# anilkeshwani/speech-integration

Measured on AMD Instinct MI355X. Metric: train_tokens_per_sec, higher is better.
Workload: dtype bf16; 1 GPU; Llama-3.2-1B +5000 DSUs (V=133258), SFT step fwd+bwd+AdamW, seq_len=2048, batch=8/GPU, grad_accum=1, 16 layers, random-init weights, MLS-shaped synthetic DSU sequences; global_batch=8, seq_len=2048, parallelism=dp1

## Files before the change

speech-integration_amd/csrc/attn_mfma.h:

```cpp
#pragma once
#include <type_traits>
#include "common_hip.h"

namespace {

__device__ __forceinline__ bf16x4 unrope4(bf16x4 v, f32x4 cs) {
    const float x0 = (float)v[0], x1 = (float)v[1], x2 = (float)v[2], x3 = (float)v[3];
    bf16x4 o;
    o[0] = (bf16_t)(x0 * cs[0] + x1 * cs[1]);
    o[1] = (bf16_t)(x1 * cs[0] - x0 * cs[1]);
    o[2] = (bf16_t)(x2 * cs[2] + x3 * cs[3]);
    o[3] = (bf16_t)(x3 * cs[2] - x2 * cs[3]);
    return o;
}
__device__ __forceinline__ bf16x4 unrope4(bf16x4 v, const float* __restrict__ tb, int d0) {
    return unrope4(v, *reinterpret_cast<const f32x4*>(tb + d0));
}

__device__ __forceinline__ void block_to_work(int n_blocks, int n_pairs, int& rank, int& pair) {
    const int i = (int)blockIdx.x;
    if (n_pairs % 8 == 0) {
        const int ppx = n_pairs / 8, xcd = i & 7, j = i >> 3;
        rank = j / ppx;
        pair = xcd * ppx + j % ppx;
    } else {
        rank = i % n_blocks;
        pair = i / n_blocks;
    }
}

__device__ __forceinline__ void ring_barrier() { asm volatile("s_waitcnt lgkmcnt(0)\n\ts_barrier" ::: "memory"); }

#ifdef ATTN_TRACE
constexpr int TRACE_MAX = 8192;
__device__ unsigned long long g_attn_trace[3][TRACE_MAX][6];
#define TRACE_BEGIN() const unsigned long long tr_t0_ = __builtin_amdgcn_s_memrealtime(); unsigned long long tr_ta_ = 0, tr_tb_ = 0
#define TRACE_LOOP_BEGIN() tr_ta_ = __builtin_amdgcn_s_memrealtime()
#define TRACE_LOOP_END() tr_tb_ = __builtin_amdgcn_s_memrealtime()
#define TRACE_END(k, work)                                                                                                        \
    if (threadIdx.x == 0 && blockIdx.x < TRACE_MAX) {                                                                             \
        unsigned hw_, xcc_;                                                                                                       \
        asm volatile("s_getreg_b32 %0, hwreg(HW_REG_HW_ID)" : "=s"(hw_));                                                        \
        asm volatile("s_getreg_b32 %0, hwreg(HW_REG_XCC_ID)" : "=s"(xcc_));                                                      \
        g_attn_trace[k][blockIdx.x][0] = tr_t0_;                                                                                  \
        g_attn_trace[k][blockIdx.x][1] = __builtin_amdgcn_s_memrealtime();                                                        \
        g_attn_trace[k][blockIdx.x][2] = ((unsigned long long)xcc_ << 32) | hw_;                                                  \
        g_attn_trace[k][blockIdx.x][3] = (unsigned long long)(work);                                                              \
        g_attn_trace[k][blockIdx.x][4] = tr_ta_;                                                                                  \
        g_attn_trace[k][blockIdx.x][5] = tr_tb_;                                                                                  \
    }
#else
#define TRACE_BEGIN()
#define TRACE_LOOP_BEGIN()
#define TRACE_LOOP_END()
#define TRACE_END(k, work)
#endif

constexpr int HD = 64;
constexpr float LOG2E = 1.4426950408889634f;

__device__ __forceinline__ int rowmap(int r, int h) { return (r & 3) + 8 * (r >> 2) + 4 * h; }

enum { SWZ_ROW = 0, SWZ_TR = 1, SWZ_DUAL = 2 };
template <int SWZ> __device__ __forceinline__ int swz(int row) {
    if (SWZ == SWZ_ROW) return (row >> 1) & 7;
    if (SWZ == SWZ_TR) return ((row >> 1) & 1) << 2;
    return (((row >> 1) & 1) << 2) | ((row >> 2) & 3);
}

template <int SWZ> __device__ __forceinline__ bf16x8 frag_row(const char* tile, int row_base, int ks, int lane) {
    const int row = row_base + (lane & 31);
    const int chunk = (2 * ks + (lane >> 5)) ^ swz<SWZ>(row);
    return *reinterpret_cast<const bf16x8*>(tile + row * 128 + chunk * 16);
}

template <int SWZ> __device__ __forceinline__ bf16x8 frag_tr(const char* tile, int kbase, int cbase, int lane) {
    const int G = lane >> 4, h = G >> 1, i = lane & 15, q = i >> 2, p = i & 3;
    const int chunk = ((cbase + 16 * (G & 1)) >> 3) + (p >> 1);
    const int r0 = kbase + 4 * h + q, r1 = r0 + 8;
    const char* a0 = tile + r0 * 128 + ((chunk ^ swz<SWZ>(r0)) * 16) + 8 * (p & 1);
    const char* a1 = tile + r1 * 128 + ((chunk ^ swz<SWZ>(r1)) * 16) + 8 * (p & 1);
    s16x4 lo = __builtin_amdgcn_ds_read_tr16_b64_v4i16((__attribute__((address_space(3))) s16x4*)a0);
    s16x4 hi = __builtin_amdgcn_ds_read_tr16_b64_v4i16((__attribute__((address_space(3))) s16x4*)a1);
    typedef __attribute__((ext_vector_type(8))) short s16x8;
    s16x8 r = __builtin_shufflevector(lo, hi, 0, 1, 2, 3, 4, 5, 6, 7);
    return __builtin_bit_cast(bf16x8, r);
}

template <int SWZ> __device__ __forceinline__ s16x4 frag_tr_half(const char* tile, int kbase, int cbase, int lane, int half) {
    const int G = lane >> 4, h = G >> 1, i = lane & 15, q = i >> 2, p = i & 3;
    const int chunk = ((cbase + 16 * (G & 1)) >> 3) + (p >> 1);
    const int r = kbase + 4 * h + q + 8 * half;
    const char* a = tile + r * 128 + ((chunk ^ swz<SWZ>(r)) * 16) + 8 * (p & 1);
    return __builtin_amdgcn_ds_read_tr16_b64_v4i16((__attribute__((address_space(3))) s16x4*)a);
}

__device__ __forceinline__ bf16x8 acc_frag(const f32x16& a, int s) {
    bf16x8 f;
#pragma unroll
    for (int j = 0; j < 8; ++j) f[j] = (bf16_t)a[8 * s + j];
    return f;
}

__device__ __forceinline__ bf16x8 scale_frag(bf16x8 v, float s) {
#pragma unroll
    for (int j = 0; j < 8; ++j) v[j] = (bf16_t)((float)v[j] * s);
    return v;
}

template <int ROWS, int NTHR> struct TileStage {
    static constexpr int N = ROWS * 8 / NTHR;
    u32x4 r[N];
    __device__ __forceinline__ void load(const bf16_t* g, int64_t ld, int tid) {
#pragma unroll
        for (int i = 0; i < N; ++i) {
            const int c = tid + i * NTHR;
            r[i] = *reinterpret_cast<const u32x4*>(g + (int64_t)(c >> 3) * ld + (c & 7) * 8);
        }
    }
    template <int SWZ> __device__ __forceinline__ void store(char* tile, int tid) const {
#pragma unroll
        for (int i = 0; i < N; ++i) {
            const int c = tid + i * NTHR, row = c >> 3, chunk = (c & 7) ^ swz<SWZ>(row);
            *reinterpret_cast<u32x4*>(tile + row * 128 + chunk * 16) = r[i];
        }
    }
};

typedef __attribute__((address_space(3))) char lds_c;
constexpr unsigned BUF_RSRC_WORD3 = 0x00020000u;
__device__ __forceinline__ u32x4 buffer_rsrc(const void* base) {
    const uint64_t a = (uint64_t)(uintptr_t)base;
    u32x4 r;
    r[0] = __builtin_amdgcn_readfirstlane((unsigned)a);
    r[1] = __builtin_amdgcn_readfirstlane((unsigned)(a >> 32) & 0xffffu);
    r[2] = 0x7fffffffu;
    r[3] = BUF_RSRC_WORD3;
    return r;
}
__device__ __forceinline__ void dma16(unsigned lds_dst, unsigned voff, u32x4 rs, unsigned soff) {
    asm volatile("s_mov_b32 m0, %0\n\ts_nop 0\n\tbuffer_load_dwordx4 %1, %2, %3 offen lds" ::"s"(lds_dst), "v"(voff), "s"(rs), "s"(soff) : "memory");
}
__device__ __forceinline__ void dma4(unsigned lds_dst, unsigned voff, u32x4 rs, unsigned soff) {
    asm volatile("s_mov_b32 m0, %0\n\ts_nop 0\n\tbuffer_load_dword %1, %2, %3 offen lds" ::"s"(lds_dst), "v"(voff), "s"(rs), "s"(soff) : "memory");
}

#ifndef ATTN_NW
#define ATTN_NW 4
#endif
constexpr int ANW = ATTN_NW, ANP = 8 / ATTN_NW;
template <int SWZ_K, int SWZ_V> struct KvTileDma {
    u32x4 rs;
    unsigned vk[ANP], vv[ANP];
    unsigned lds_piece;
    unsigned tile_bytes;
    __device__ __forceinline__ void init(const bf16_t* kbase, int64_t ld, int kv_cols, const char* smem, int wave, int lane) {
        rs = buffer_rsrc(kbase);
#pragma unroll
        for (int p = 0; p < ANP; ++p) {
            const int row = (p * ANW + wave) * 8 + (lane >> 3);
            vk[p] = (unsigned)((row * ld + ((lane & 7) ^ swz<SWZ_K>(row)) * 8) * 2);
            vv[p] = (unsigned)((row * ld + kv_cols + ((lane & 7) ^ swz<SWZ_V>(row)) * 8) * 2);
        }
        lds_piece = __builtin_amdgcn_readfirstlane((unsigned)(uintptr_t)(lds_c*)smem + (unsigned)wave * 1024u);
        tile_bytes = (unsigned)(64 * ld * 2);
    }
    __device__ __forceinline__ void tile(int t, unsigned slot_bytes) const {
        const unsigned soff = (unsigned)t * tile_bytes;
#pragma unroll
        for (int p = 0; p < ANP; ++p) {
            dma16(lds_piece + slot_bytes + p * ANW * 1024, vk[p], rs, soff);
            dma16(lds_piece + slot_bytes + 8192 + p * ANW * 1024, vv[p], rs, soff);
        }
    }
    __device__ __forceinline__ void piece(int t, unsigned slot_bytes, int i) const {
        const unsigned soff = (unsigned)t * tile_bytes;
        const int p = i >> 1;
        if (i & 1) dma16(lds_piece + slot_bytes + 8192 + p * ANW * 1024, vv[p], rs, soff);
        else dma16(lds_piece + slot_bytes + p * ANW * 1024, vk[p], rs, soff);
    }
};

struct RowTileDma {
    u32x4 rs;
    unsigned voff[2];
    unsigned step;
    __device__ __forceinline__ void init(const bf16_t* base, int64_t ld, int lane) {
        rs = buffer_rsrc(base);
#pragma unroll
        for (int par = 0; par < 2; ++par)
            voff[par] = (unsigned)(((lane >> 3) * ld + ((lane & 7) ^ (lane >> 4) ^ (4 * par)) * 8) * 2);
        step = (unsigned)(8 * ld * 2);
    }
    __device__ __forceinline__ void request(int i, unsigned lds_tile) const { dma16(lds_tile + i * 1024, voff[i & 1], rs, (unsigned)i * step); }
};

__device__ __forceinline__ unsigned pack_bf16(float a, float b) {
    typedef __attribute__((ext_vector_type(2))) __bf16 bf16x2_;
    bf16x2_ v;
    v[0] = (bf16_t)a;
    v[1] = (bf16_t)b;
    return __builtin_bit_cast(unsigned, v);
}

}

struct AttnBwdArgs {
    const void* qkv; int64_t ld; const void *out, *dout; const float* lse; void* dqkv; float* delta;
    const int32_t *doc_start, *doc_end; const float* rope; int64_t table_len; const int32_t* positions;
    int64_t batch, seq; int n_heads, n_kv; void* workspace; int64_t workspace_bytes;
    const int32_t *plan_dev, *plan_header;
    hipStream_t stream;
};
```

speech-integration_amd/csrc/common_hip.h:

```cpp
#pragma once
#include <hip/hip_runtime.h>
#include <stdint.h>
#include <stdio.h>
#include "../../include/ssi_hip.h"

typedef __bf16 bf16_t;
typedef __attribute__((ext_vector_type(2))) float f32x2;
typedef __attribute__((ext_vector_type(4))) float f32x4;
typedef __attribute__((ext_vector_type(16))) float f32x16;
typedef __attribute__((ext_vector_type(4))) __bf16 bf16x4;
typedef __attribute__((ext_vector_type(8))) __bf16 bf16x8;
typedef __attribute__((ext_vector_type(4))) short s16x4;
typedef __attribute__((ext_vector_type(4))) unsigned int u32x4;
typedef __attribute__((ext_vector_type(2))) unsigned int u32x2;

#define SSI_WAVE 64

void ssi_set_error(const char* fmt, ...);

#define SSI_CHECK_ARG(cond)                                                                  \
    do {                                                                                     \
        if (!(cond)) {                                                                       \
            ssi_set_error("%s:%d: argument check failed: %s", __FILE__, __LINE__, #cond);    \
            return SSI_ERR_ARG;                                                              \
        }                                                                                    \
    } while (0)

#define SSI_LAUNCH_CHECK()                                                                   \
    do {                                                                                     \
        hipError_t e_ = hipGetLastError();                                                   \
        if (e_ != hipSuccess) {                                                              \
            ssi_set_error("%s:%d: launch failed: %s", __FILE__, __LINE__, hipGetErrorString(e_)); \
            return SSI_ERR_HIP + (int)e_;                                                    \
        }                                                                                    \
    } while (0)

static inline int64_t ssi_cdiv(int64_t a, int64_t b) { return (a + b - 1) / b; }
static inline int64_t ssi_align_up(int64_t a, int64_t b) { return ssi_cdiv(a, b) * b; }

template <typename T> __device__ __forceinline__ float to_f32(T v);
template <> __device__ __forceinline__ float to_f32<float>(float v) { return v; }
template <> __device__ __forceinline__ float to_f32<bf16_t>(bf16_t v) { return (float)v; }
template <typename T> __device__ __forceinline__ T from_f32(float v);
template <> __device__ __forceinline__ float from_f32<float>(float v) { return v; }
template <> __device__ __forceinline__ bf16_t from_f32<bf16_t>(float v) { return (bf16_t)v; }

template <typename T> __device__ __forceinline__ float ssi_sigmoid(float x);
template <> __device__ __forceinline__ float ssi_sigmoid<float>(float x) { return 1.f / (1.f + expf(-x)); }
template <> __device__ __forceinline__ float ssi_sigmoid<bf16_t>(float x) {
    return __builtin_amdgcn_rcpf(1.f + __builtin_amdgcn_exp2f(x * -1.44269504088896f));
}
template <typename T> __device__ __forceinline__ float ssi_silu(float x);
template <> __device__ __forceinline__ float ssi_silu<float>(float x) { return x / (1.f + expf(-x)); }
template <> __device__ __forceinline__ float ssi_silu<bf16_t>(float x) { return x * ssi_sigmoid<bf16_t>(x); }
template <typename T> __device__ __forceinline__ void ssi_swiglu_bwd_elem(float gf, float uf, float df, float& dgate, float& dup) {
#pragma clang fp contract(off)
    const float sig = ssi_sigmoid<T>(gf);
    const float one_minus = 1.f - sig;
    const float t = 1.f + gf * one_minus;
    dup = df * (gf * sig);
    dgate = (df * uf) * (sig * t);
}

__device__ __forceinline__ void ssi_rope_pair(float x0, float x1, float c, float s, float& o0, float& o1) {
#pragma clang fp contract(off)
    o0 = x0 * c - x1 * s;
    o1 = x1 * c + x0 * s;
}

template <typename T> struct Vec16;
template <> struct Vec16<float> {
    static constexpr int N = 4;
    f32x4 v;
    __device__ __forceinline__ float get(int i) const { return v[i]; }
    __device__ __forceinline__ void set(int i, float x) { v[i] = x; }
};
template <> struct Vec16<bf16_t> {
    static constexpr int N = 8;
    bf16x8 v;
    __device__ __forceinline__ float get(int i) const { return (float)v[i]; }
    __device__ __forceinline__ void set(int i, float x) { v[i] = (bf16_t)x; }
};
template <typename T> __device__ __forceinline__ Vec16<T> load16(const T* p) {
    Vec16<T> r;
    r.v = *reinterpret_cast<const decltype(r.v)*>(p);
    return r;
}
template <typename T> __device__ __forceinline__ void store16(T* p, const Vec16<T>& r) {
    *reinterpret_cast<decltype(r.v)*>(p) = r.v;
}

template <typename T> __device__ __forceinline__ Vec16<T> load16_nt(const T* p) {
    Vec16<T> r;
    r.v = __builtin_nontemporal_load(reinterpret_cast<const decltype(r.v)*>(p));
    return r;
}
template <typename T> __device__ __forceinline__ void store16_nt(T* p, const Vec16<T>& r) {
    __builtin_nontemporal_store(r.v, reinterpret_cast<decltype(r.v)*>(p));
}

__device__ __forceinline__ float wave_sum(float v) {
#pragma unroll
    for (int o = 32; o > 0; o >>= 1) v += __shfl_xor(v, o, 64);
    return v;
}
__device__ __forceinline__ float wave_max(float v) {
#pragma unroll
    for (int o = 32; o > 0; o >>= 1) v = fmaxf(v, __shfl_xor(v, o, 64));
    return v;
}
__device__ __forceinline__ float block_sum(float v, float* red) {
    v = wave_sum(v);
    const int w = threadIdx.x >> 6, l = threadIdx.x & 63, nw = (blockDim.x + 63) >> 6;
    __syncthreads();
    if (l == 0) red[w] = v;
    __syncthreads();
    float t = (l < nw) ? red[l] : 0.f;
    t = wave_sum(t);
    return t;
}
__device__ __forceinline__ float block_max(float v, float* red) {
    v = wave_max(v);
    const int w = threadIdx.x >> 6, l = threadIdx.x & 63, nw = (blockDim.x + 63) >> 6;
    __syncthreads();
    if (l == 0) red[w] = v;
    __syncthreads();
    float t = (l < nw) ? red[l] : -INFINITY;
    t = wave_max(t);
    return t;
}

template <bool ENABLED, int N, bool FENCED = false> struct PhaseStamps {
    unsigned long long begin = __builtin_readcyclecounter(), last = begin, total[N] = {};
    __device__ __forceinline__ void reset() {
        if (FENCED) __builtin_amdgcn_sched_barrier(0);
        last = __builtin_readcyclecounter();
        if (FENCED) __builtin_amdgcn_sched_barrier(0);
    }
    __device__ __forceinline__ void tick(int i) {
        const unsigned long long prev = last;
        reset();
        total[i] += last - prev;
    }
};
template <int N, bool FENCED> struct PhaseStamps<false, N, FENCED> {
    __device__ __forceinline__ void reset() {}
    __device__ __forceinline__ void tick(int) {}
};

int ssi_get_impl();

bool ssi_gemm_mfma_supported(int layout, int64_t M, int64_t N, int64_t K, const void* A, int64_t lda, const void* B,
                             int64_t ldb, const void* C, int64_t ldc, const void* R);
int ssi_gemm_mfma_bf16(int layout, int64_t M, int64_t N, int64_t K, const void* A, int64_t lda, const void* B,
                       int64_t ldb, void* C, int64_t ldc, const void* R, float alpha, const float* alpha_dev,
                       int accumulate, void* stream);
int ssi_gemm_mfma_bf16_splitk(int layout, int64_t M, int64_t N, int64_t K, const void* A, int64_t lda, const void* B,
                              int64_t ldb, void* C, int64_t ldc, const void* R, float alpha, const float* alpha_dev,
                              int accumulate, int splits, float* slabs, void* stream);
bool ssi_gemm_mfma_bf16_batched(int layout, int batch, int64_t M, int64_t N, int64_t K, const void* A, int64_t lda, int64_t bsA, const void* B,
                                int64_t ldb, int64_t bsB, void* C, int64_t ldc, int64_t bsC, float alpha, const float* alpha_dev, int accumulate,
                                void* stream, int* rc);
void ssi_gemm_mfma_set_dynamic_tiles(int on);
bool ssi_gemm_rope_mfma(int64_t M, int64_t N, int64_t K, const void* A, int64_t lda, const void* B, int64_t ldb, void* C, int64_t ldc,
                        const float* rope, const int32_t* positions, int64_t seq, int64_t rot_cols, void* stream, int* rc);
bool ssi_gemm_swiglu_supported(int64_t M, int64_t inter, int64_t K, const void* p0, const void* p1, const void* p2, const void* p3,
                               int64_t ld0, int64_t ld1, int64_t ld2, int64_t ld3);
int ssi_gemm_swiglu_fwd_mfma(int64_t M, int64_t inter, int64_t K, const void* X, int64_t ldx, const void* W13, int64_t ldw,
                             void* GU, int64_t ldgu, void* ACT, int64_t ldact, void* stream);
int ssi_gemm_swiglu_bwd_mfma(int layout, int64_t M, int64_t inter, int64_t K, const void* DY, int64_t lddy, const void* W2, int64_t ldw,
                             const void* GU, int64_t ldgu, void* DGU, int64_t lddgu, void* stream);
bool ssi_gemm_swiglu_bwd_nn_supported(int64_t K, int64_t lddy, int64_t ldw);

bool ssi_gemm_f32_mfma_supported(int layout, int64_t M, int64_t N, int64_t K, const void* A, int64_t lda, const void* B,
                                 int64_t ldb, const void* C, int64_t ldc, const void* R);
int ssi_gemm_f32_mfma(int layout, int64_t M, int64_t N, int64_t K, const void* A, int64_t lda, const void* B, int64_t ldb,
                      void* C, int64_t ldc, const void* R, float alpha, const float* alpha_dev, int accumulate,
                      void* stream);

bool ssi_attn_mfma_supported(int64_t ld, int64_t batch, int64_t seq, int n_heads, int n_kv, int head_dim, int dtype);
void ssi_attn_note_dispatch(int v);
int ssi_attn_bwd_mfma(const void* qkv, int64_t ld, const void* out, const void* dout, const float* lse, void* dqkv,
                      float* delta, const int32_t* doc_start, const int32_t* doc_end, const float* rope, int64_t table_len,
                      const int32_t* positions, int64_t batch, int64_t seq, int n_heads, int n_kv, void* workspace, int64_t workspace_bytes,
                      const int32_t* plan_dev, const int32_t* host_plan_header, void* stream);
int ssi_attn_fwd_mfma(const void* qkv, int64_t ld, void* out, float* lse, const int32_t* doc_start, int64_t batch, int64_t seq,
                      int n_heads, int n_kv, void* stream);
int64_t ssi_attn_mfma_bwd_workspace_bytes(int64_t batch, int64_t seq, int n_heads, int n_kv);

#define SSI_DISPATCH_DTYPE(dtype, ...)                           \
    do {                                                         \
        if ((dtype) == SSI_F32) {                                \
            using T = float;                                     \
            __VA_ARGS__;                                         \
        } else if ((dtype) == SSI_BF16) {                        \
            using T = bf16_t;                                    \
            __VA_ARGS__;                                         \
        } else {                                                 \
            ssi_set_error("unsupported dtype %d", (int)(dtype)); \
            return SSI_ERR_ARG;                                  \
        }                                                        \
    } while (0)
```

speech-integration_amd/csrc/embed_ce.hip:

```cpp
#include "common_hip.h"

template <typename T>
__global__ __launch_bounds__(256) void embed_fwd_kernel(const int64_t* __restrict__ tokens, const T* __restrict__ table,
                                                        T* __restrict__ out, int64_t n_tok, int dim, int64_t vocab) {
    constexpr int N = Vec16<T>::N;
    const int nvec = dim / N;
    for (int64_t t = blockIdx.x; t < n_tok; t += gridDim.x) {
        const int64_t tok = tokens[t];
        const bool ok = tok >= 0 && tok < vocab;
        for (int v = threadIdx.x; v < nvec; v += 256) {
            Vec16<T> a;
            if (ok) a = load16(table + tok * dim + v * N);
            else
#pragma unroll
                for (int i = 0; i < N; ++i) a.set(i, 0.f);
            store16(out + t * dim + v * N, a);
        }
    }
}

extern "C" int ssi_embed_fwd(const int64_t* tokens, const void* table, void* out, int64_t n_tok, int64_t dim,
                             int64_t vocab, int dtype, void* stream) {
    if (n_tok == 0) return SSI_OK;
    SSI_CHECK_ARG(tokens && table && out && n_tok > 0 && dim > 0 && dim % 8 == 0 && vocab > 0);
    const unsigned grid = (unsigned)(n_tok < 65536 ? n_tok : 65536);
    SSI_DISPATCH_DTYPE(dtype, hipLaunchKernelGGL(embed_fwd_kernel<T>, dim3(grid), dim3(256), 0, (hipStream_t)stream, tokens,
                                                 (const T*)table, (T*)out, n_tok, (int)dim, vocab));
    SSI_LAUNCH_CHECK();
    return SSI_OK;
}

__global__ __launch_bounds__(256) void embed_index_kernel(const int64_t* __restrict__ tokens, int64_t n_tok, int64_t vocab,
                                                          int* __restrict__ first, int* __restrict__ count) {
    const int64_t t = (int64_t)blockIdx.x * 256 + threadIdx.x;
    if (t >= n_tok) return;
    const int64_t tok = tokens[t];
    if (tok < 0 || tok >= vocab) return;
    atomicMin(&first[tok], (int)t);
    atomicAdd(&count[tok], 1);
}

template <typename T, int MAXV>
__global__ __launch_bounds__(256) void embed_bwd_kernel(const int64_t* __restrict__ tokens, const T* __restrict__ dout,
                                                        T* __restrict__ dtable, int64_t n_tok, int dim, int64_t vocab,
                                                        const int* __restrict__ first, const int* __restrict__ count) {
    constexpr int N = Vec16<T>::N;
    const int lane = threadIdx.x & 63;
    const int64_t t0 = (int64_t)blockIdx.x * 4 + (threadIdx.x >> 6);
    if (t0 >= n_tok) return;
    const int64_t tok = tokens[t0];
    if (tok < 0 || tok >= vocab) return;
    if (first[tok] != (int)t0) return;
    const int need = count[tok];
    const int nvec = dim / N;
    float acc[MAXV][N];
#pragma unroll
    for (int k = 0; k < MAXV; ++k)
#pragma unroll
        for (int i = 0; i < N; ++i) acc[k][i] = 0.f;
    constexpr int SCAN = 8, ROWS = 8;
    __shared__ int hits_lds[4][64 * SCAN];
    int* hits = hits_lds[threadIdx.x >> 6];
    int found = 0;
    for (int64_t base0 = (t0 / 64) * 64; base0 < n_tok && found < need; base0 += 64 * SCAN) {
        int64_t tk[SCAN];
#pragma unroll
        for (int u = 0; u < SCAN; ++u) {
            const int64_t idx = base0 + 64 * u + lane;
            tk[u] = tokens[idx < n_tok ? idx : n_tok - 1];
        }
        int n = 0;
#pragma unroll
        for (int u = 0; u < SCAN; ++u) {
            const int64_t idx = base0 + 64 * u + lane;
            const bool hit = idx < n_tok && idx >= t0 && tk[u] == tok;
            const unsigned long long mask = __ballot(hit);
            if (hit) hits[n + __popcll(mask & ((1ull << lane) - 1ull))] = (int)(idx - base0);
            n += __popcll(mask);
        }
        __builtin_amdgcn_s_waitcnt(0xc07f);
        if (n == 1) {
            const T* src = dout + (base0 + hits[0]) * dim;
#pragma unroll
            for (int k = 0; k < MAXV; ++k) {
                const int v = lane + k * 64;
                const Vec16<T> r = load16(src + (v < nvec ? v : nvec - 1) * N);
#pragma unroll
                for (int i = 0; i < N; ++i) acc[k][i] += v < nvec ? r.get(i) : 0.f;
            }
        } else
        for (int h0 = 0; h0 < n; h0 += ROWS) {
            int pos[ROWS];
#pragma unroll
            for (int u = 0; u < ROWS; ++u) pos[u] = hits[h0 + u < n ? h0 + u : n - 1];
            Vec16<T> a[ROWS][MAXV];
#pragma unroll
            for (int u = 0; u < ROWS; ++u) {
                const T* src = dout + (base0 + pos[u]) * dim;
#pragma unroll
                for (int k = 0; k < MAXV; ++k) {
                    const int v = lane + k * 64;
                    a[u][k] = load16(src + (v < nvec ? v : nvec - 1) * N);
                }
            }
            __builtin_amdgcn_sched_barrier(0);
#pragma unroll
            for (int u = 0; u < ROWS; ++u) {
                const bool row_ok = h0 + u < n;
#pragma unroll
                for (int k = 0; k < MAXV; ++k) {
                    const bool ok = row_ok && lane + k * 64 < nvec;
#pragma unroll
                    for (int i = 0; i < N; ++i) acc[k][i] += ok ? a[u][k].get(i) : 0.f;
                }
            }
        }
        found += n;
    }
    T* dst = dtable + tok * dim;
#pragma unroll
    for (int k = 0; k < MAXV; ++k) {
        const int v = lane + k * 64;
        if (v < nvec) {
            Vec16<T> a = load16(dst + v * N);
#pragma unroll
            for (int i = 0; i < N; ++i) a.set(i, a.get(i) + acc[k][i]);
            store16(dst + v * N, a);
        }
    }
}

static inline int64_t embed_ws_vocab_slots(int64_t vocab) { return ssi_align_up(vocab, 64); }
extern "C" int64_t ssi_embed_bwd_workspace_bytes(int64_t vocab) { return 2 * embed_ws_vocab_slots(vocab) * (int64_t)sizeof(int); }

template <typename T>
static int launch_embed_bwd(const int64_t* tokens, const T* dout, T* dtable, int64_t n_tok, int dim, int64_t vocab,
                            const int* first, const int* count, hipStream_t st) {
    const int64_t vec_per_lane = ssi_cdiv(dim / Vec16<T>::N, 64);
    const dim3 grid((unsigned)ssi_cdiv(n_tok, 4));
    if (vec_per_lane <= 1) hipLaunchKernelGGL((embed_bwd_kernel<T, 1>), grid, dim3(256), 0, st, tokens, dout, dtable, n_tok, dim, vocab, first, count);
    else if (vec_per_lane <= 2) hipLaunchKernelGGL((embed_bwd_kernel<T, 2>), grid, dim3(256), 0, st, tokens, dout, dtable, n_tok, dim, vocab, first, count);
    else if (vec_per_lane <= 4) hipLaunchKernelGGL((embed_bwd_kernel<T, 4>), grid, dim3(256), 0, st, tokens, dout, dtable, n_tok, dim, vocab, first, count);
    else if (vec_per_lane <= 8) hipLaunchKernelGGL((embed_bwd_kernel<T, 8>), grid, dim3(256), 0, st, tokens, dout, dtable, n_tok, dim, vocab, first, count);
    else { ssi_set_error("embed_bwd: dim %d too large", dim); return SSI_ERR_UNSUPPORTED; }
    return SSI_OK;
}

extern "C" int ssi_embed_bwd(const int64_t* tokens, const void* dout, void* dtable, int64_t n_tok, int64_t dim,
                             int64_t vocab, int dtype, void* workspace, int64_t workspace_bytes, void* stream) {
    if (n_tok == 0) return SSI_OK;
    SSI_CHECK_ARG(tokens && dout && dtable && n_tok > 0 && n_tok < (1LL << 31) && dim > 0 && dim % 8 == 0 && vocab > 0);
    if (!workspace || workspace_bytes < ssi_embed_bwd_workspace_bytes(vocab)) { ssi_set_error("embed_bwd: workspace too small"); return SSI_ERR_WORKSPACE; }
    auto st = (hipStream_t)stream;
    int* first = (int*)workspace;
    int* count = first + embed_ws_vocab_slots(vocab);
    hipError_t e = hipMemsetAsync(first, 0x7f, embed_ws_vocab_slots(vocab) * sizeof(int), st);
    if (e == hipSuccess) e = hipMemsetAsync(count, 0, embed_ws_vocab_slots(vocab) * sizeof(int), st);
    if (e != hipSuccess) { ssi_set_error("embed_bwd: memset failed: %s", hipGetErrorString(e)); return SSI_ERR_HIP + (int)e; }
    hipLaunchKernelGGL(embed_index_kernel, dim3((unsigned)ssi_cdiv(n_tok, 256)), dim3(256), 0, st, tokens, n_tok, vocab, first, count);
    SSI_LAUNCH_CHECK();
    int rc = SSI_OK;
    SSI_DISPATCH_DTYPE(dtype, rc = launch_embed_bwd<T>(tokens, (const T*)dout, (T*)dtable, n_tok, (int)dim, vocab, first, count, st));
    if (rc) return rc;
    SSI_LAUNCH_CHECK();
    return SSI_OK;
}

template <typename T>
__global__ __launch_bounds__(512) void ce_fwd_kernel(T* __restrict__ logits, int64_t ld, const int64_t* __restrict__ labels,
                                                     int64_t vocab, int64_t ignore_index, float* __restrict__ row_loss,
                                                     float* __restrict__ row_lse, int write_grad, const float* __restrict__ row_weight) {
    constexpr int N = Vec16<T>::N;
    __shared__ float red[16];
    const int64_t row = blockIdx.x;
    T* lr = logits + row * ld;
    const int64_t label = labels[row];
    const bool valid = label != ignore_index && label >= 0 && label < vocab;
    const int64_t nvec = ld / N;
    if (!valid) {
        if (threadIdx.x == 0) { row_loss[row] = 0.f; if (row_lse) row_lse[row] = 0.f; }
        if (write_grad) {
            Vec16<T> z;
#pragma unroll
            for (int i = 0; i < N; ++i) z.set(i, 0.f);
            for (int64_t v = threadIdx.x; v < nvec; v += 512) store16(lr + v * N, z);
        }
        return;
    }
    float m = -INFINITY, s = 0.f;
    for (int64_t v = threadIdx.x; v < nvec; v += 512) {
        Vec16<T> a = load16(lr + v * N);
        float lm = -INFINITY;
#pragma unroll
        for (int i = 0; i < N; ++i) if (v * N + i < vocab) lm = fmaxf(lm, a.get(i));
        if (lm > m) { s *= expf(m - lm); m = lm; }
#pragma unroll
        for (int i = 0; i < N; ++i) if (v * N + i < vocab) s += expf(a.get(i) - m);
    }
    const float gm = block_max(m, red);
    s = (m == -INFINITY) ? 0.f : s * expf(m - gm);
    const float gs = block_sum(s, red);
    const float lse = gm + logf(gs);
    const float w = row_weight ? row_weight[row] : 1.f;
    if (threadIdx.x == 0) {
        row_loss[row] = w * (lse - to_f32<T>(lr[label]));
        if (row_lse) row_lse[row] = lse;
    }
    if (!write_grad) return;
    __syncthreads();
    for (int64_t v = threadIdx.x; v < nvec; v += 512) {
        Vec16<T> a = load16(lr + v * N), o;
#pragma unroll
        for (int i = 0; i < N; ++i) {
            const int64_t c = v * N + i;
            float g = 0.f;
            if (c < vocab) g = w * (expf(a.get(i) - lse) - (c == label ? 1.f : 0.f));
            o.set(i, g);
        }
        store16(lr + v * N, o);
    }
}

template <int NCH, bool write_grad>
__global__ __launch_bounds__(1024, 4) void ce_row_bf16_kernel(bf16_t* __restrict__ logits, int64_t ld, const int64_t* __restrict__ labels,
                                                              int64_t rows, int64_t vocab, int64_t ignore_index,
                                                              float* __restrict__ row_loss, float* __restrict__ row_lse,
                                                              const float* __restrict__ row_weight) {
    __shared__ float red[16];
    constexpr float LOG2E = 1.44269504088896340736f;
    constexpr int CHUNK = 8192;
    const int tid = threadIdx.x;
    const int voff = tid * 16;
    const int col0 = tid * 8;
    const int row_bytes = (int)(ld * 2);
    const int vocab_i = (int)vocab;
    u32x4 x[NCH];
    auto is_valid = [&](int64_t label) { return label != ignore_index && label >= 0 && label < vocab; };
    auto rsrc_of = [&](int64_t row) { return __builtin_amdgcn_make_buffer_rsrc(logits + row * ld, 0, row_bytes, 0x00020000u); };
    auto lo = [](unsigned u) { return __builtin_bit_cast(float, u << 16); };
    auto hi = [](unsigned u) { return __builtin_bit_cast(float, u & 0xffff0000u); };
    auto opaque = [&]() {
#pragma unroll
        for (int c = 0; c < NCH; ++c)
#pragma unroll
            for (int d = 0; d < 4; ++d) asm volatile("" : "+v"(x[c][d]));
    };
    int64_t row = blockIdx.x;
    if (row >= rows) return;
    {
        const __amdgpu_buffer_rsrc_t r0 = rsrc_of(row);
#pragma unroll
        for (int c = 0; c < NCH; ++c) x[c] = __builtin_amdgcn_raw_buffer_load_b128(r0, voff, c * CHUNK * 2, 0);
    }
    for (; row < rows; row += gridDim.x) {
        const int64_t next = row + gridDim.x;
        const int64_t label = labels[row];
        const bool valid = is_valid(label);
        const float w = row_weight ? row_weight[row] : 1.f;
        const float log2w = row_weight ? __log2f(w) : 0.f;
        const __amdgpu_buffer_rsrc_t rs = rsrc_of(row);
#pragma unroll
        for (int c = (NCH >= 2 ? NCH - 2 : 0); c < NCH; ++c) {
            const int left = vocab_i - c * CHUNK - col0;
#pragma unroll
            for (int d = 0; d < 4; ++d) {
                if (2 * d >= left) x[c][d] = (x[c][d] & 0xffff0000u) | 0x0000ff80u;
                if (2 * d + 1 >= left) x[c][d] = (x[c][d] & 0x0000ffffu) | 0xff800000u;
            }
        }
        float nl = -INFINITY;
        if (valid) {
            float xl = 0.f;
            if (tid == 0) xl = (float)logits[row * ld + label];
            float m = -INFINITY;
#pragma unroll
            for (int c = 0; c < NCH; ++c)
#pragma unroll
                for (int d = 0; d < 4; ++d) m = fmaxf(m, fmaxf(lo(x[c][d]), hi(x[c][d])));
            asm volatile("s_waitcnt vmcnt(0)" ::: "memory");
            const float gm = block_max(m, red);
            opaque();
            const float nm = -gm * LOG2E;
            float s = 0.f;
#pragma unroll
            for (int c = 0; c < NCH; ++c)
#pragma unroll
                for (int d = 0; d < 4; ++d)
                    s += __builtin_amdgcn_exp2f(fmaf(lo(x[c][d]), LOG2E, nm)) + __builtin_amdgcn_exp2f(fmaf(hi(x[c][d]), LOG2E, nm));
            const float gs = block_sum(s, red);
            const float lse = gm + logf(gs);
            if (tid == 0) {
                row_loss[row] = w * (lse - xl);
                if (row_lse) row_lse[row] = lse;
            }
            nl = -lse * LOG2E + log2w;
        } else if (tid == 0) {
            row_loss[row] = 0.f;
            if (row_lse) row_lse[row] = 0.f;
        }
        opaque();
        const int hot = valid ? (int)label - col0 : -(1 << 30);
        const __amdgpu_buffer_rsrc_t rn = rsrc_of(next < rows ? next : row);
#pragma unroll
        for (int c = 0; c < NCH; ++c) {
            if (write_grad) {
                float g[8];
#pragma unroll
                for (int d = 0; d < 4; ++d) {
                    g[2 * d] = __builtin_amdgcn_exp2f(fmaf(lo(x[c][d]), LOG2E, nl));
                    g[2 * d + 1] = __builtin_amdgcn_exp2f(fmaf(hi(x[c][d]), LOG2E, nl));
                }
                const int h = hot - c * CHUNK;
                if ((unsigned)h < 8u) {
#pragma unroll
                    for (int e = 0; e < 8; ++e) if (e == h) g[e] -= w;
                }
                bf16x8 ob;
#pragma unroll
                for (int e = 0; e < 8; ++e) ob[e] = (bf16_t)g[e];
                __builtin_amdgcn_raw_buffer_store_b128(__builtin_bit_cast(u32x4, ob), rs, voff, c * CHUNK * 2, 2 );
            }
            x[c] = __builtin_amdgcn_raw_buffer_load_b128(rn, voff, c * CHUNK * 2, 2 );
            __builtin_amdgcn_sched_barrier(0);
        }
    }
}

static int ce_num_cus() {
    static const int n = [] {
        int dev = 0, cus = 0;
        if (hipGetDevice(&dev) != hipSuccess || hipDeviceGetAttribute(&cus, hipDeviceAttributeMultiprocessorCount, dev) != hipSuccess || cus <= 0) cus = 256;
        return cus;
    }();
    return n;
}

extern "C" int ssi_ce_fwd_weighted(void* logits, int64_t ld, const int64_t* labels, const float* row_weight, int64_t rows, int64_t vocab,
                                   int64_t ignore_index, float* row_loss, float* row_lse, int write_grad, int dtype, void* stream) {
    SSI_CHECK_ARG(logits && labels && row_loss && rows >= 0 && vocab > 0 && ld >= vocab && ld % 8 == 0);
    if (rows == 0) return SSI_OK;
    const int64_t chunks = ssi_cdiv(ld, 8192);
    const bool row_form = dtype == SSI_BF16 && ((uintptr_t)logits & 15) == 0 && ld - vocab < 8192 && ld * 2 < (1LL << 31) &&
                          (chunks <= 4 || chunks == 8 || (chunks >= 16 && chunks <= 18));
    if (row_form) {
        const dim3 grid((unsigned)(rows < ce_num_cus() ? rows : ce_num_cus()));
#define SSI_CE_ROW(N)                                                                                                                       \
    case N:                                                                                                                                 \
        if (write_grad) hipLaunchKernelGGL((ce_row_bf16_kernel<N, true>), grid, dim3(1024), 0, (hipStream_t)stream, (bf16_t*)logits, ld, labels, \
                                           rows, vocab, ignore_index, row_loss, row_lse, row_weight);                                       \
        else hipLaunchKernelGGL((ce_row_bf16_kernel<N, false>), grid, dim3(1024), 0, (hipStream_t)stream, (bf16_t*)logits, ld, labels, rows,     \
                                vocab, ignore_index, row_loss, row_lse, row_weight);                                                        \
        break
        switch ((int)chunks) {
            SSI_CE_ROW(1); SSI_CE_ROW(2); SSI_CE_ROW(3); SSI_CE_ROW(4); SSI_CE_ROW(8); SSI_CE_ROW(16); SSI_CE_ROW(17); SSI_CE_ROW(18);
        }
#undef SSI_CE_ROW
        SSI_LAUNCH_CHECK();
        return SSI_OK;
    }
    SSI_DISPATCH_DTYPE(dtype, hipLaunchKernelGGL(ce_fwd_kernel<T>, dim3((unsigned)rows), dim3(512), 0, (hipStream_t)stream,
                                                 (T*)logits, ld, labels, vocab, ignore_index, row_loss, row_lse, write_grad, row_weight));
    SSI_LAUNCH_CHECK();
    return SSI_OK;
}

extern "C" int ssi_ce_fwd(void* logits, int64_t ld, const int64_t* labels, int64_t rows, int64_t vocab,
                          int64_t ignore_index, float* row_loss, float* row_lse, int write_grad, int dtype, void* stream) {
    return ssi_ce_fwd_weighted(logits, ld, labels, nullptr, rows, vocab, ignore_index, row_loss, row_lse, write_grad, dtype, stream);
}

__global__ __launch_bounds__(1024) void ce_reduce_kernel(const float* __restrict__ row_loss, const int64_t* __restrict__ labels,
                                                         int64_t rows, int64_t vocab, int64_t ignore_index, float* __restrict__ out) {
    __shared__ float red[16];
    float s = 0.f, c = 0.f, bad = 0.f;
    for (int64_t r = threadIdx.x; r < rows; r += 1024) {
        const int64_t l = labels[r];
        const bool in_range = l >= 0 && l < vocab;
        if (l != ignore_index && in_range) { s += row_loss[r]; c += 1.f; }
        else if (l != ignore_index) bad += 1.f;
    }
    s = block_sum(s, red);
    c = block_sum(c, red);
    bad = block_sum(bad, red);
    if (threadIdx.x == 0) { out[0] = s / c; out[1] = s; out[2] = c; out[3] = bad; }
}

extern "C" int ssi_ce_reduce(const float* row_loss, const int64_t* labels, int64_t rows, int64_t vocab, int64_t ignore_index,
                             float* out, void* stream) {
    SSI_CHECK_ARG(row_loss && labels && out && rows >= 0 && rows < (1LL << 24) && vocab > 0);
    hipLaunchKernelGGL(ce_reduce_kernel, dim3(1), dim3(1024), 0, (hipStream_t)stream, row_loss, labels, rows, vocab, ignore_index, out);
    SSI_LAUNCH_CHECK();
    return SSI_OK;
}
```

Measured before the change: 159,500 tokens/s.

## Prefetch next CE row into LDS via buffer-load DMA during softmax

In the fused cross-entropy row kernel, once the block max is known the next row's logits chunks are requested straight into LDS with buffer_load...lds DMA. The grad-writing loop then reads those chunks from LDS instead of issuing global loads after each store. The goal is to overlap fetching the next row with the exp/sum and gradient-write phases. The DMA helpers move to common_hip.h and buffer_rsrc gains a size argument. The cost is up to 144KB of LDS per block, which could limit occupancy, plus hand-written vmcnt waits that must count in-flight loads correctly.

```diff
diff --git a/speech-integration_amd/csrc/attn_mfma.h b/speech-integration_amd/csrc/attn_mfma.h
--- a/speech-integration_amd/csrc/attn_mfma.h
+++ b/speech-integration_amd/csrc/attn_mfma.h
@@ -127,24 +127,6 @@
     }
 };
 
-typedef __attribute__((address_space(3))) char lds_c;
-constexpr unsigned BUF_RSRC_WORD3 = 0x00020000u;
-__device__ __forceinline__ u32x4 buffer_rsrc(const void* base) {
-    const uint64_t a = (uint64_t)(uintptr_t)base;
-    u32x4 r;
-    r[0] = __builtin_amdgcn_readfirstlane((unsigned)a);
-    r[1] = __builtin_amdgcn_readfirstlane((unsigned)(a >> 32) & 0xffffu);
-    r[2] = 0x7fffffffu;
-    r[3] = BUF_RSRC_WORD3;
-    return r;
-}
-__device__ __forceinline__ void dma16(unsigned lds_dst, unsigned voff, u32x4 rs, unsigned soff) {
-    asm volatile("s_mov_b32 m0, %0\n\ts_nop 0\n\tbuffer_load_dwordx4 %1, %2, %3 offen lds" ::"s"(lds_dst), "v"(voff), "s"(rs), "s"(soff) : "memory");
-}
-__device__ __forceinline__ void dma4(unsigned lds_dst, unsigned voff, u32x4 rs, unsigned soff) {
-    asm volatile("s_mov_b32 m0, %0\n\ts_nop 0\n\tbuffer_load_dword %1, %2, %3 offen lds" ::"s"(lds_dst), "v"(voff), "s"(rs), "s"(soff) : "memory");
-}
-
 #ifndef ATTN_NW
 #define ATTN_NW 4
 #endif
diff --git a/speech-integration_amd/csrc/common_hip.h b/speech-integration_amd/csrc/common_hip.h
--- a/speech-integration_amd/csrc/common_hip.h
+++ b/speech-integration_amd/csrc/common_hip.h
@@ -147,6 +147,24 @@
     __device__ __forceinline__ void reset() {}
     __device__ __forceinline__ void tick(int) {}
 };
+
+typedef __attribute__((address_space(3))) char lds_c;
+constexpr unsigned BUF_RSRC_WORD3 = 0x00020000u;
+__device__ __forceinline__ u32x4 buffer_rsrc(const void* base, unsigned bytes = 0x7fffffffu) {
+    const uint64_t a = (uint64_t)(uintptr_t)base;
+    u32x4 r;
+    r[0] = __builtin_amdgcn_readfirstlane((unsigned)a);
+    r[1] = __builtin_amdgcn_readfirstlane((unsigned)(a >> 32) & 0xffffu);
+    r[2] = bytes;
+    r[3] = BUF_RSRC_WORD3;
+    return r;
+}
+__device__ __forceinline__ void dma16(unsigned lds_dst, unsigned voff, u32x4 rs, unsigned soff) {
+    asm volatile("s_mov_b32 m0, %0\n\ts_nop 0\n\tbuffer_load_dwordx4 %1, %2, %3 offen lds" ::"s"(lds_dst), "v"(voff), "s"(rs), "s"(soff) : "memory");
+}
+__device__ __forceinline__ void dma4(unsigned lds_dst, unsigned voff, u32x4 rs, unsigned soff) {
+    asm volatile("s_mov_b32 m0, %0\n\ts_nop 0\n\tbuffer_load_dword %1, %2, %3 offen lds" ::"s"(lds_dst), "v"(voff), "s"(rs), "s"(soff) : "memory");
+}
 
 int ssi_get_impl();
 
diff --git a/speech-integration_amd/csrc/embed_ce.hip b/speech-integration_amd/csrc/embed_ce.hip
--- a/speech-integration_amd/csrc/embed_ce.hip
+++ b/speech-integration_amd/csrc/embed_ce.hip
@@ -221,12 +221,18 @@
     }
 }
 
+#ifndef CE_LDS_SLOTS
+#define CE_LDS_SLOTS 9
+#endif
+constexpr int CE_SLOT_BYTES = 16384;
 template <int NCH, bool write_grad>
 __global__ __launch_bounds__(1024, 4) void ce_row_bf16_kernel(bf16_t* __restrict__ logits, int64_t ld, const int64_t* __restrict__ labels,
                                                               int64_t rows, int64_t vocab, int64_t ignore_index,
                                                               float* __restrict__ row_loss, float* __restrict__ row_lse,
                                                               const float* __restrict__ row_weight) {
+    constexpr int P = !write_grad ? 0 : NCH < CE_LDS_SLOTS ? NCH : CE_LDS_SLOTS;
     __shared__ float red[16];
+    __shared__ __attribute__((aligned(16))) char land[P > 0 ? P * CE_SLOT_BYTES : 16];
     constexpr float LOG2E = 1.44269504088896340736f;
     constexpr int CHUNK = 8192;
     const int tid = threadIdx.x;
@@ -245,6 +251,15 @@
 #pragma unroll
             for (int d = 0; d < 4; ++d) asm volatile("" : "+v"(x[c][d]));
     };
+    const unsigned land_wave = __builtin_amdgcn_readfirstlane((unsigned)(uintptr_t)(lds_c*)land + (unsigned)(tid >> 6) * 1024u);
+    auto request_next = [&](int64_t next) __attribute__((always_inline)) {
+        if (P > 0 && next < rows) {
+            const u32x4 rq = buffer_rsrc(logits + next * ld, (unsigned)row_bytes);
+            asm volatile("s_waitcnt lgkmcnt(0)" ::: "memory");
+#pragma unroll
+            for (int c = 0; c < P; ++c) dma16(land_wave + (unsigned)(c * CE_SLOT_BYTES), (unsigned)voff, rq, (unsigned)(c * CHUNK * 2));
+        }
+    };
     int64_t row = blockIdx.x;
     if (row >= rows) return;
     {
@@ -252,6 +267,7 @@
 #pragma unroll
         for (int c = 0; c < NCH; ++c) x[c] = __builtin_amdgcn_raw_buffer_load_b128(r0, voff, c * CHUNK * 2, 0);
     }
+    if (P > 0) opaque();
     for (; row < rows; row += gridDim.x) {
         const int64_t next = row + gridDim.x;
         const int64_t label = labels[row];
@@ -279,6 +295,7 @@
                 for (int d = 0; d < 4; ++d) m = fmaxf(m, fmaxf(lo(x[c][d]), hi(x[c][d])));
             asm volatile("s_waitcnt vmcnt(0)" ::: "memory");
             const float gm = block_max(m, red);
+            request_next(next);
             opaque();
             const float nm = -gm * LOG2E;
             float s = 0.f;
@@ -294,9 +311,12 @@
                 if (row_lse) row_lse[row] = lse;
             }
             nl = -lse * LOG2E + log2w;
-        } else if (tid == 0) {
-            row_loss[row] = 0.f;
-            if (row_lse) row_lse[row] = 0.f;
+        } else {
+            request_next(next);
+            if (tid == 0) {
+                row_loss[row] = 0.f;
+                if (row_lse) row_lse[row] = 0.f;
+            }
         }
         opaque();
         const int hot = valid ? (int)label - col0 : -(1 << 30);
@@ -320,10 +340,16 @@
                 for (int e = 0; e < 8; ++e) ob[e] = (bf16_t)g[e];
                 __builtin_amdgcn_raw_buffer_store_b128(__builtin_bit_cast(u32x4, ob), rs, voff, c * CHUNK * 2, 2 );
             }
-            x[c] = __builtin_amdgcn_raw_buffer_load_b128(rn, voff, c * CHUNK * 2, 2 );
+            if (c < P) {
+                asm volatile("s_waitcnt vmcnt(%0)" ::"n"(P) : "memory");
+                x[c] = *reinterpret_cast<const u32x4*>(land + c * CE_SLOT_BYTES + voff);
+            } else {
+                x[c] = __builtin_amdgcn_raw_buffer_load_b128(rn, voff, c * CHUNK * 2, 2 );
+            }
             __builtin_amdgcn_sched_barrier(0);
         }
     }
+    if (P > 0) asm volatile("s_waitcnt vmcnt(0)" ::: "memory");
 }
 
 static int ce_num_cus() {
```

Result: no change. 159,300 tokens/s (median of 3 runs) (-0.1%).
